# alshai/Big-BWT

Measured on AMD Instinct MI355X. Metric: input MB/s to .bwt (bit-exact vs ref), higher is better.
Workload: dtype u8; 1 GPU; BASELINE configs[2]: 64x mutated yeast-shaped FASTA (~0.79 GB), -w 10 -p 100, BWT + -s -e sampled SA; bytes_per_gpu=787308470, w=10, p=100, flags=6, phrases=16409159, words=921010, dict_bytes=79900101, parallelism=1 GPU

## Files before the change

big-bwt_amd/csrc/sufsort.hip:

```cpp
#include "kernels.hpp"
#include "prims.hpp"
#include "devutil.hpp"
#include <algorithm>
#include <cmath>
#include <optional>
#include <vector>
#include <cstdio>
#include <cstdlib>

namespace pfp {

enum : int { MODE_DICT = 0, MODE_PLAIN = 1 };

struct SufGeom {
  int mode; uint64_t N; WordView wv;
  const uint32_t *sym = nullptr;
  const uint32_t *dist = nullptr;
};
__device__ __forceinline__ uint64_t suf_len(const SufGeom &g, uint64_t i) {
  if (g.mode == MODE_DICT) return slen_of(g.wv, i) + 1;
  return g.N - i;
}

struct KeyCode {
// ... 529 lines not shown
#pragma unroll
      for (int s = 0; s < B; s++)
        if ((uint32_t)s < steps && !done) {
          const uint32_t qs = q + 4 * (uint32_t)s;
          differ(qs, X[s].x, Y[s].x); differ(qs + 1, X[s].y, Y[s].y); differ(qs + 2, X[s].z, Y[s].z); differ(qs + 3, X[s].w, Y[s].w);
        }
      q += 4 * steps;
    }
  }
  key[a] = k;
  val[a] = (I)i;
}
template <class I>
__global__ void heads64seg_kernel(uint64_t m, const uint8_t *__restrict__ gs, const uint64_t *__restrict__ key,
                                  const I *__restrict__ aslot, uint8_t *__restrict__ hd, I *__restrict__ hv) {
  uint64_t a = (uint64_t)BID * blockDim.x + threadIdx.x;
  if (a >= m) return;
  bool h = gs[a] || key[a] != key[a - 1];
  hd[a] = h ? 1 : 0;
  hv[a] = h ? aslot[a] : (I)0;
}
__global__ void rare_marks_kernel(const uint32_t *__restrict__ s, uint32_t N, const uint32_t *__restrict__ occ, uint32_t n_sym,
                                  uint32_t below, uint32_t *__restrict__ v) {
  uint32_t j = BID * blockDim.x + threadIdx.x;
  if (j >= N) return;
  const uint32_t x = s[N - 1 - j];
  const bool rare = x == 0 || x > n_sym || occ[x - 1] < below;
  v[j] = rare ? j + 1 : 0u;
}
__global__ void rare_dist_kernel(uint32_t N, const uint32_t *__restrict__ pm, uint32_t *__restrict__ dist) {
  uint32_t i = BID * blockDim.x + threadIdx.x;
  if (i >= N) return;
  const uint32_t j = N - 1 - i, mk = pm[j];
  dist[i] = mk ? j + 1 - mk : 0xFFFFFFFFu;
}

constexpr int kTile = 256;
__global__ __launch_bounds__(256) void active_count_kernel(const uint8_t *__restrict__ keep, const uint8_t *__restrict__ hd,
                                                           uint64_t m, uint32_t *__restrict__ tile_keep,
                                                           uint32_t *__restrict__ tile_heads) {
  const uint64_t t = (uint64_t)BID * 256 + threadIdx.x;
  const uint64_t base = t * 16;
  uint32_t k[4] = {0, 0, 0, 0}, h[4] = {0, 0, 0, 0};
  if (base < m) { load_flags16(keep, base, m, k); load_flags16(hd, base, m, h); }
  uint32_t ck = __popc(k[0]) + __popc(k[1]) + __popc(k[2]) + __popc(k[3]);
  uint32_t ch = __popc(k[0] & h[0]) + __popc(k[1] & h[1]) + __popc(k[2] & h[2]) + __popc(k[3] & h[3]);
#pragma unroll
  for (int o = 8; o > 0; o >>= 1) { ck += __shfl_down(ck, o, 16); ch += __shfl_down(ch, o, 16); }
  if ((threadIdx.x & 15) == 0 && base < m) { tile_keep[t >> 4] = ck; tile_heads[t >> 4] = ch; }
}
template <class I>
__global__ __launch_bounds__(256) void active_place_kernel(const uint8_t *__restrict__ keep, uint64_t m,
                                                           const uint32_t *__restrict__ tile_keep,
                                                           const I *__restrict__ tile_off,
                                                           const I *__restrict__ aslot, const I *__restrict__ val,
                                                           const I *__restrict__ newhead, I finbit,
                                                           I *__restrict__ aslot2, I *__restrict__ act_i,
                                                           I *__restrict__ act_grp) {
  __shared__ uint32_t ws[4];
  if ((uint64_t)BID * kTile >= m) return;
  if (tile_keep[BID] == 0) return;
  const uint64_t a = (uint64_t)BID * kTile + threadIdx.x;
  const bool k = a < m && keep[a];
  const unsigned long long mask = __ballot(k);
  const int lane = threadIdx.x & 63, wv = threadIdx.x >> 6;
  if (lane == 0) ws[wv] = (uint32_t)__popcll(mask);
  __syncthreads();
  if (!k) return;
  I pos = tile_off[BID] + (I)__popcll(mask & ((1ull << lane) - 1ull));
  for (int q = 0; q < wv; q++) pos += ws[q];
  aslot2[pos] = aslot ? aslot[a] : (I)a; act_i[pos] = val[a] & ~finbit; act_grp[pos] = newhead[a];
}

template <class I, class K>
__global__ void heads_kernel(uint64_t m, const K *__restrict__ key, const I *__restrict__ aslot,
                             uint8_t *__restrict__ hd, I *__restrict__ hv) {
  uint64_t a = (uint64_t)BID * blockDim.x + threadIdx.x;
  if (a >= m) return;
  bool h = (a == 0) || key[a] != key[a - 1];
  hd[a] = h ? 1 : 0;
  hv[a] = h ? aslot[a] : (I)0;
}

template <class I>
__global__ __launch_bounds__(256) void heads0_kernel(uint64_t m, const uint64_t *__restrict__ key, uint64_t keymask, int shift,
                                                     uint32_t T, uint8_t *__restrict__ hd, I *__restrict__ tile_last,
                                                     I *__restrict__ tab) {
  __shared__ I wl[4];
  if ((uint64_t)BID * 256 >= m) return;
  const uint64_t a = (uint64_t)BID * 256 + threadIdx.x;
  bool h = false;
  if (a < m) {
    const uint64_t k = key[a] & keymask, kprev = a ? (key[a - 1] & keymask) : ~k;
    h = k != kprev;
    hd[a] = h ? 1 : 0;
    if (a == 0 || (k >> shift) != (kprev >> shift)) tab[T - 1 - (uint32_t)(k >> shift)] = IdxTraits<I>::kNone - (I)a;
  }
  const unsigned long long mask = __ballot(h);
  if ((threadIdx.x & 63) == 0)
    wl[threadIdx.x >> 6] = mask ? (I)(BID * 256ull + (threadIdx.x & ~63) + (63 - __clzll((long long)mask))) : (I)0;
  __syncthreads();
  if (threadIdx.x == 0) {
    I v = wl[0];
    for (int q = 1; q < 4; q++) v = wl[q] > v ? wl[q] : v;
    tile_last[BID] = v;
  }
}
template <class I>
__global__ void fill_kernel(I *p, uint64_t n, I v) {
  uint64_t i = (uint64_t)BID * blockDim.x + threadIdx.x;
  if (i < n) p[i] = v;
}
template <class I>
__global__ __launch_bounds__(256) void write_back0_kernel(uint64_t m, const I *__restrict__ val,
                                                          const I *__restrict__ tile_scan,
                                                          const uint8_t *__restrict__ hd, const uint64_t *__restrict__ key0,
                                                          I *__restrict__ rank,
                                                          I *__restrict__ grp, uint8_t *__restrict__ keep, int write_ranks) {
  __shared__ I wl[4];
  if ((uint64_t)BID * 256 >= m) return;
  const uint64_t a = (uint64_t)BID * 256 + threadIdx.x;
  const int lane = threadIdx.x & 63, wv = threadIdx.x >> 6;
  const bool in = a < m;
  const bool h = in && hd[a];
  const bool hnext = in && (a + 1 == m || hd[a + 1]);
  const I i = in ? val[a] : (I)0;
  const uint32_t flagbit = in ? (uint32_t)(key0[a] & 1ull) : 0u;
  const I carry = BID ? tile_scan[BID - 1] : (I)0;
  const unsigned long long mask = __ballot(h);
  const I wbase = (I)(BID * 256ull + (threadIdx.x & ~63));
  if (lane == 0) wl[wv] = mask ? wbase + (63 - __clzll((long long)mask)) : (I)0;
  __syncthreads();
  if (!in) return;
  const unsigned long long upto = mask & (~0ull >> (63 - lane));
  I head;
  if (upto) head = wbase + (63 - __clzll((long long)upto));
  else {
    head = carry;
    for (int q = 0; q < wv; q++) head = wl[q] > head ? wl[q] : head;
  }
  grp[a] = head;
  const bool single = h && hnext;
  const bool fin = !single && flagbit;
  const bool k = !single && !fin;
  if (k && write_ranks) rank[i] = head;
  keep[a] = k ? 1 : 0;
}

template <class I>
__global__ void scatter_settled_kernel(uint64_t N, const I *__restrict__ sa, const I *__restrict__ grp,
                                       const uint8_t *__restrict__ keep, I finbit, I *__restrict__ rank) {
  uint64_t t = (uint64_t)BID * blockDim.x + threadIdx.x;
  if (t < N && !keep[t]) rank[sa[t]] = grp[t] | finbit;
}

constexpr int kPivBits = 23;
constexpr uint32_t kPivEq = 1u << 21;
constexpr uint32_t kPivCapMax = 8192;
template <class I>
__global__ void build_keys_pivot_kernel(const uint8_t *__restrict__ s, uint64_t m, uint64_t from, uint32_t cap,
                                        const I *__restrict__ act_i, const I *__restrict__ act_grp,
                                        const I *__restrict__ sa, I finbit, uint64_t *__restrict__ key,
                                        uint32_t *__restrict__ key32, I *__restrict__ val, int both = 0) {
  uint64_t a = (uint64_t)BID * blockDim.x + threadIdx.x;
  if (a >= m) return;
  const I i = act_i[a], grp = act_grp[a];
  const I piv = sa[grp];
  uint32_t ok = kPivEq;
  I settled = finbit;
  if (i != piv) {
    settled = 0;
    const uint8_t *pa = s + i + from, *pp = s + piv + from;
    uint32_t off = 0;
    uint4 xa0, xa1, xp0, xp1;
    bool hit = false;
    for (; off < cap; off += 32) {
      xa0 = ld16u(pa + off); xa1 = ld16u(pa + off + 16); xp0 = ld16u(pp + off); xp1 = ld16u(pp + off + 16);
      const uint32_t diff = (xa0.x ^ xp0.x) | (xa0.y ^ xp0.y) | (xa0.z ^ xp0.z) | (xa0.w ^ xp0.w) | (xa1.x ^ xp1.x) |
                            (xa1.y ^ xp1.y) | (xa1.z ^ xp1.z) | (xa1.w ^ xp1.w);
      const uint32_t term = lt2_flags32(xa0.x) | lt2_flags32(xa0.y) | lt2_flags32(xa0.z) | lt2_flags32(xa0.w) | lt2_flags32(xa1.x) |
                            lt2_flags32(xa1.y) | lt2_flags32(xa1.z) | lt2_flags32(xa1.w);
      if (diff | term) { hit = true; break; }
    }
    if (hit) {
      const uint64_t x[4] = {(uint64_t)xa0.x | ((uint64_t)xa0.y << 32), (uint64_t)xa0.z | ((uint64_t)xa0.w << 32),
                             (uint64_t)xa1.x | ((uint64_t)xa1.y << 32), (uint64_t)xa1.z | ((uint64_t)xa1.w << 32)};
      const uint64_t y[4] = {(uint64_t)xp0.x | ((uint64_t)xp0.y << 32), (uint64_t)xp0.z | ((uint64_t)xp0.w << 32),
                             (uint64_t)xp1.x | ((uint64_t)xp1.y << 32), (uint64_t)xp1.z | ((uint64_t)xp1.w << 32)};
      bool done = false;
#pragma unroll
      for (int q = 0; q < 4 && !done; q++) {
        const uint64_t tb = lt2_flags64(x[q]);
        if (x[q] == y[q]) { if (tb) { settled = finbit; done = true; } continue; }
        const int fd = __builtin_ctzll(x[q] ^ y[q]) >> 3;
        const int ft = tb ? (__builtin_ctzll(tb) >> 3) : 8;
        if (ft < fd) { settled = finbit; done = true; continue; }
        const uint32_t bx = (uint32_t)(x[q] >> (8 * fd)) & 0xffu, by = (uint32_t)(y[q] >> (8 * fd)) & 0xffu;
        const uint32_t lcp = off + 8 * q + fd;
        ok = bx < by ? ((lcp << 8) | bx) : ((2u << 21) | ((kPivCapMax - 1 - lcp) << 8) | bx);
        if (bx <= kEndOfWord) settled = finbit;
        done = true;
      }
    }
  }
  if (key32) key32[a] = ok;
  if (!key32 || both) key[a] = ((uint64_t)grp << kPivBits) | ok;
  val[a] = i | settled;
}
template <class I>
__global__ void veto_clear_kernel(uint64_t m, const I *__restrict__ newhead, uint8_t *__restrict__ veto) {
  uint64_t a = (uint64_t)BID * blockDim.x + threadIdx.x;
  if (a < m) veto[newhead[a]] = 0;
}
template <class I>
__global__ void pivot_veto_kernel(uint64_t m, const uint64_t *__restrict__ key, const uint32_t *__restrict__ key32,
                                  const I *__restrict__ val, const I *__restrict__ newhead, I finbit,
                                  uint8_t *__restrict__ veto) {
  uint64_t a = (uint64_t)BID * blockDim.x + threadIdx.x;
  if (a >= m) return;
  const uint32_t ok = key32 ? key32[a] : ((uint32_t)key[a] & ((1u << kPivBits) - 1));
  if (ok == kPivEq && !(val[a] & finbit)) veto[newhead[a]] = 1;
}

template <class I, class K>
__global__ void write_back_kernel(SufGeom g, uint64_t m, uint64_t sorted_len, const I *__restrict__ aslot,
                                  const I *__restrict__ val, const I *__restrict__ newhead,
                                  const uint8_t *__restrict__ hd, I finbit, const K *__restrict__ prevkey,
                                  int prevshift, const I *__restrict__ prevgrp, const uint8_t *__restrict__ veto,
                                  const uint32_t *__restrict__ wstart_bits, I *__restrict__ sa,
                                  I *__restrict__ rank, I *__restrict__ wordrank, I *__restrict__ grp, uint8_t *__restrict__ keep) {
  uint64_t a = (uint64_t)BID * blockDim.x + threadIdx.x;
  if (a >= m) return;
  const I iv = val[a], i = iv & ~finbit;
  const I slot = aslot[a];
  sa[slot] = i;
  grp[slot] = newhead[a];
// ... 38 lines not shown
                                    const I *__restrict__ sa, const I *__restrict__ grp, I finbit,
                                    I *__restrict__ rank) {
  uint64_t t = (uint64_t)BID * blockDim.x + threadIdx.x;
  if (t < N && refined[t] && !active[t]) rank[sa[t]] = grp[t] | finbit;
}

constexpr uint64_t kFinishMax = 1u << 17;
constexpr int kFinishGrp = 64;
constexpr uint32_t kFinishCmp = 8192;
__device__ __forceinline__ int finish_cmp_dict(const uint8_t *__restrict__ s, uint64_t i, uint64_t j, uint32_t *ovf) {
  for (uint32_t k = 0; k < kFinishCmp; k += 8) {
    const int r = cmp_term8(ld8u(s + i + k), ld8u(s + j + k));
    if (r != kCmpOn) return r;
  }
  *ovf = 1;
  return 0;
}
__device__ __forceinline__ int finish_cmp_int(const uint32_t *__restrict__ sym, uint64_t i, uint64_t j, uint32_t *ovf) {
  for (uint32_t k = 0; k < kFinishCmp / 4; k++) {
    const uint32_t x = sym[i + k], y = sym[j + k];
    if (x != y) return x < y ? -1 : 1;
  }
  *ovf = 1;
  return 0;
}
template <class I>
__global__ void finish_rank_kernel(SufGeom g, const uint8_t *__restrict__ s, uint64_t m, const I *__restrict__ act_i,
                                   const I *__restrict__ act_grp, uint32_t *__restrict__ lt, uint32_t *__restrict__ eq,
                                   uint32_t *__restrict__ gstart, uint32_t *__restrict__ overflow) {
  const uint64_t t = (uint64_t)BID * blockDim.x + threadIdx.x;
  const uint64_t a = t >> 3;
  const int l8 = (int)(t & 7);
  if (a >= m) return;
  const I grp = act_grp[a];
  uint64_t gs = a, ge = a + 1;
  while (gs > 0 && a - gs < (uint64_t)kFinishGrp && act_grp[gs - 1] == grp) gs--;
  while (ge < m && ge - gs <= (uint64_t)kFinishGrp && act_grp[ge] == grp) ge++;
  if (ge - gs > (uint64_t)kFinishGrp || (gs > 0 && act_grp[gs - 1] == grp)) { if (l8 == 0) atomicOr(overflow, 1u); return; }
  const uint64_t ia = act_i[a];
  uint32_t nlt = 0, neq = 0, ovf = 0;
  for (uint64_t b = gs + (uint64_t)l8; b < ge; b += 8) {
    if (b == a) continue;
    if (*(volatile uint32_t *)overflow) break;
    const uint64_t ib = act_i[b];
    const int cmp = g.mode == MODE_DICT ? finish_cmp_dict(s, ib, ia, &ovf) : finish_cmp_int(g.sym, ib, ia, &ovf);
    if (cmp < 0) nlt++;
    else if (cmp == 0 && b < a) neq++;
  }
  uint32_t packed = nlt | (neq << 8) | (ovf << 16);
  packed += __shfl_xor(packed, 1, 64); packed += __shfl_xor(packed, 2, 64); packed += __shfl_xor(packed, 4, 64);
  if (l8 != 0) return;
  if (packed >> 16) atomicOr(overflow, 1u);
  lt[a] = packed & 0xffu; eq[a] = (packed >> 8) & 0xffu; gstart[a] = (uint32_t)gs;
}
template <class I>
__global__ void finish_write_kernel(SufGeom g, uint64_t m, const I *__restrict__ aslot, const I *__restrict__ act_i, const uint32_t *__restrict__ lt,
                                    const uint32_t *__restrict__ eq, const uint32_t *__restrict__ gstart, I finbit,
                                    I *__restrict__ sa, I *__restrict__ grp, I *__restrict__ rank, I *__restrict__ wordrank) {
  const uint64_t a = (uint64_t)BID * blockDim.x + threadIdx.x;
  if (a >= m) return;
  const uint64_t gs = gstart[a];
  const I i = act_i[a], slot = aslot[gs + lt[a] + eq[a]], head = aslot[gs + lt[a]];
  sa[slot] = i;
  grp[slot] = head;
  if (rank) rank[i] = head | finbit;
  else if (wordrank && ((uint64_t)i == 0 || g.wv.bytes[(uint64_t)i - 1] == kEndOfWord)) wordrank[word_of(g.wv, i)] = head | finbit;
}

constexpr uint32_t kPivotAvg = 1024u;

constexpr uint64_t kLazyRatio = 8ull;

constexpr uint32_t kSegMinAvg = 24u;

struct SorterSwitches {
  bool lib_sort = getenv("PFP_OWN_SORT") == nullptr;
  bool finflag = getenv("PFP_NO_FINFLAG") == nullptr;
  bool finisher = getenv("PFP_NO_FINISHER") == nullptr;
  bool small_seg = getenv("PFP_NO_SMALLSEG") == nullptr;
  bool trace_rounds = getenv("PFP_TRACE_ROUNDS") != nullptr;
  uint32_t pivot_cap = []() { const char *e = getenv("PFP_PIVOT_CAP"); uint32_t v = e ? (uint32_t)atoll(e) : 512u; return v > kPivCapMax ? kPivCapMax : v; }();
};
static const SorterSwitches kSwitch;

template <class I>
RankViewT<I> rank_view(const SuffixOrderT<I> &so) {
  return RankViewT<I>{so.rank.p, so.skeys.p, so.tab.p, so.lut.p, so.bytes, so.N, so.kbits, so.shift, so.T, so.finbit, so.keymask, so.wordrank.p};
}
template RankViewT<uint32_t> rank_view(const SuffixOrderT<uint32_t> &);
template RankViewT<uint64_t> rank_view(const SuffixOrderT<uint64_t> &);

struct DoublingOpts {
  int key_bits = 64;
  bool dict = false;
  std::optional<uint64_t> list_len;
  bool whole_list = false;
  int idx_bits = 0;
};

enum class Round {
  FirstDict,
  FirstPlain,
  DictPivotGlobal,
  DictPivotGrouped,
  ParsePivot,
  DoublingGlobal,
  DoublingGrouped,
};

template <class I>
struct Rounds {
  using K = typename IdxTraits<I>::DKey;
  static constexpr bool kWide = sizeof(I) == 8;
  static constexpr int TB = 256;

  pfp_ctx *const c;
  const SufGeom g;
  SuffixOrderT<I> &out;
  const DoublingOpts o;
  const uint64_t NP, N;
  const bool lazy;
  const bool list_mode;
  const bool range_mode;
  const int nb;
  bool lazy_active = false, late_rank = false;
  I *rank_p = nullptr, *wordrank_p = nullptr;

  Round kind;
  uint64_t m, h, m2 = 0, ngrp = 0;
  uint32_t piv_cap = kSwitch.pivot_cap;
  bool pivot_ok = true;
  bool ipiv_ok = true;
  bool small_failed = false;
  bool finisher_ok = true;
  bool rank_alloc = false;
  bool lazy_pending = false;
  bool ranks_stale = false;
  bool active_stale = false;

  DBuf<uint64_t> &key;
  DBuf<I> &val;
  DBuf<I> tile_last, tile_scan;
  DBuf<uint64_t> keyo;
  DBuf<I> valo;
  DBuf<uint8_t> hd, keep;
  DBuf<I> aslot, aslot2, hv, newhead, act_i, act_grp;
  uint64_t list_cap = 0;
  DBuf<uint32_t> tile_keep, tile_heads;
  DBuf<I> tile_off, tile_hoff;
  DBuf<uint8_t> keep0, veto;
  DBuf<uint32_t> wstart_bits;
  DBuf<uint8_t> gs, bigf;
  DBuf<uint32_t> k32, k32o, segb, sege, nseg_d, ovf_d;
  DBuf<uint64_t> nsel_d;
  DBuf<K> dkey, dkeyo;

  Rounds(pfp_ctx *c_, const SufGeom &g_, DBuf<uint64_t> &key_, DBuf<I> &val_, uint64_t h0, SuffixOrderT<I> &out_, const DoublingOpts &o_)
      : c(c_), g(g_), out(out_), o(o_), NP(g_.N), N(o_.list_len.value_or(g_.N)), lazy(o_.dict), list_mode(o_.list_len.has_value()),
        range_mode(o_.list_len.has_value() && !o_.whole_list),
        nb(bits_for(N)), kind(o_.dict ? Round::FirstDict : Round::FirstPlain), m(N), h(h0), key(key_), val(val_) {}

  static uint64_t blocks(uint64_t n) { return cdiv(n, TB); }

  void first_round_sort() {
    keyo.alloc(c, N); valo.alloc(c, N);
    SortTag first_tag(g.mode == MODE_DICT ? "dictionary, first round" : "parse, first round");
    if (o.idx_bits) {
      if (kSwitch.lib_sort) sort_keys_db(c, key, keyo, N, o.idx_bits, o.idx_bits + o.key_bits);
      else msd_sort_keys_db(c, key, keyo, N, o.idx_bits, o.idx_bits + o.key_bits);
      KScope ks(c, "pfp::split_keys_kernel", N * (16 + sizeof(I)));
      hipLaunchKernelGGL(split_keys_kernel<I>, gdim(blocks(N)), gdim(TB), 0, c->stream, key.p, N, o.idx_bits, keyo.p, valo.p);
    } else {
      if (kSwitch.lib_sort) sort_pairs_db(c, key, keyo, val, valo, N, 0, o.key_bits);
      else msd_sort_pairs_db<I>(c, key, keyo, val, valo, N, 0, o.key_bits);
      std::swap(key, keyo); std::swap(val, valo);
    }
  }

  void alloc_lists(uint64_t cap) {
    aslot.alloc(c, cap); aslot2.alloc(c, cap); hv.alloc(c, cap); newhead.alloc(c, cap); act_i.alloc(c, cap); act_grp.alloc(c, cap);
    list_cap = cap;
  }
  void alloc_rank() {
    out.rank.alloc(c, NP);
    if (lazy) PFP_HIP(hipMemsetAsync(out.rank.p, 0xff, NP * sizeof(I), c->stream));
    rank_p = out.rank.p; rank_alloc = true;
  }

  void start_rounds() {
    if (lazy) { key.release(); val.release(); }
    hd.alloc(c, N + 1); keep.alloc(c, N);
    out.grp.alloc(c, N + 8);
    if (!lazy) {
      out.sa.alloc(c, N);
      alloc_lists(N);
      hipLaunchKernelGGL(iota_kernel<I>, gdim(blocks(N)), gdim(TB), 0, c->stream, aslot.p, N);
    } else {
      const int tb = std::min(o.key_bits, std::max(8, std::min(24, bits_for(N) - 5)));
      out.shift = o.key_bits - tb;
      out.T = 1u << tb;
      out.tab.alloc(c, out.T);
      hipLaunchKernelGGL(fill_kernel<I>, gdim(blocks(out.T)), gdim(TB), 0, c->stream, out.tab.p, (uint64_t)out.T,
                         (I)(IdxTraits<I>::kNone - (I)N));
    }
    out.finbit = (g.mode == MODE_DICT && (kWide || NP < (1ull << 31)) && kSwitch.finflag) ? IdxTraits<I>::kTop : (I)0;
    lazy_active = lazy && pivot_rounds_possible();
    late_rank = !range_mode && lazy_active && !c->debug;
    if (!range_mode && !late_rank) alloc_rank();
    if (late_rank) {
      out.wordrank.alloc(c, (uint64_t)g.wv.d + 1);
      PFP_HIP(hipMemsetAsync(out.wordrank.p, 0xff, ((uint64_t)g.wv.d + 1) * sizeof(I), c->stream));
      wordrank_p = out.wordrank.p;
    }
  }
  bool pivot_rounds_possible() const {
    return g.mode == MODE_DICT && out.finbit && kSwitch.pivot_cap >= 16 && (uint64_t)nb + kPivBits <= 64;
  }

  template <class KT>
  void heads(const KT *keys, int bytes) {
    KScope ks(c, "pfp::heads_kernel", m * bytes);
    hipLaunchKernelGGL((heads_kernel<I, KT>), gdim(blocks(m)), gdim(TB), 0, c->stream, m, keys, aslot.p, hd.p, hv.p);
  }
  void heads_k32() {
    KScope ks(c, "pfp::heads32_kernel", m * 14);
    hipLaunchKernelGGL(heads32_kernel<I>, gdim(blocks(m)), gdim(TB), 0, c->stream, m, gs.p, k32o.p, aslot.p, hd.p, hv.p);
  }

  void first_dict_heads_and_write_back() {
    tile_last.alloc(c, cdiv64(m, 256)); tile_scan.alloc(c, cdiv64(m, 256));
    { KScope ks(c, "pfp::heads0_kernel", m * 13);
      hipLaunchKernelGGL(heads0_kernel<I>, gdim(blocks(m)), gdim(TB), 0, c->stream, m, keyo.p, out.keymask, out.shift, out.T,
                         hd.p, tile_last.p, out.tab.p); }
    inclusive_max<I>(c, out.tab.p, out.tab.p, out.T);
    inclusive_max<I>(c, tile_last.p, tile_scan.p, cdiv64(m, 256));
    { KScope ks(c, "pfp::write_back0_kernel", m * (4 + 4 + 1 + 8 + 4 + 1));
      hipLaunchKernelGGL(write_back0_kernel<I>, gdim(blocks(m)), gdim(TB), 0, c->stream, m, valo.p, tile_scan.p, hd.p, keyo.p,
                         rank_p, out.grp.p, keep.p, (lazy_active || range_mode) ? 0 : 1); }
    if (lazy_active) active_stale = true;
    out.skeys = std::move(keyo);
    out.sa = std::move(valo);
  }

  void heads_and_write_back() {
    const uint64_t *keys = nullptr;
    const K *dkeys = nullptr;
    const I *prevgrp = nullptr;
    const uint32_t *pivk32 = nullptr;
    bool pivot = false;
    switch (kind) {
      case Round::FirstDict: return first_dict_heads_and_write_back();
      case Round::FirstPlain: heads(keyo.p, 17); break;
      case Round::DictPivotGlobal: heads(keyo.p, 17); keys = keyo.p; pivot = true; break;
      case Round::DictPivotGrouped: heads_k32(); prevgrp = act_grp.p; pivk32 = k32o.p; pivot = true; break;
      case Round::ParsePivot: {
        KScope ks(c, "pfp::heads64seg_kernel", m * 18);
        hipLaunchKernelGGL(heads64seg_kernel<I>, gdim(blocks(m)), gdim(TB), 0, c->stream, m, gs.p, keyo.p, aslot.p, hd.p, hv.p);
        prevgrp = act_grp.p;
      } break;
      case Round::DoublingGlobal:
        if constexpr (kWide) { heads(dkeyo.p, 25); dkeys = dkeyo.p; }
        else { heads(keyo.p, 17); keys = keyo.p; }
        break;
      case Round::DoublingGrouped: heads_k32(); prevgrp = act_grp.p; break;
    }
    inclusive_max<I>(c, hv.p, newhead.p, m);
    if (pivot) {
      if (!veto.p) veto.alloc(c, N);
      hipLaunchKernelGGL(veto_clear_kernel<I>, gdim(blocks(m)), gdim(TB), 0, c->stream, m, newhead.p, veto.p);
      hipLaunchKernelGGL(pivot_veto_kernel<I>, gdim(blocks(m)), gdim(TB), 0, c->stream, m, keyo.p, pivk32, valo.p, newhead.p, out.finbit, veto.p);
    }
    KScope ks(c, "pfp::write_back_kernel", m * (13 + 4 + 13));
    if (pivot && !wstart_bits.p) {
      wstart_bits.alloc(c, cdiv64(NP, 32));
      hipLaunchKernelGGL(word_start_bits_kernel, gdim(blocks(cdiv64(NP, 32))), gdim(TB), 0, c->stream, out.bytes, NP, wstart_bits.p);
    }
    const uint8_t *vetop = pivot ? veto.p : (const uint8_t *)nullptr;
    const uint32_t *lazyb = pivot ? wstart_bits.p : (const uint32_t *)nullptr;
    if (dkeys)
      hipLaunchKernelGGL((write_back_kernel<I, K>), gdim(blocks(m)), gdim(TB), 0, c->stream, g, m, h, aslot.p, valo.p, newhead.p, hd.p,
                         out.finbit, dkeys, nb, prevgrp, vetop, lazyb, out.sa.p, rank_p, wordrank_p, out.grp.p, keep.p);
    else
      hipLaunchKernelGGL((write_back_kernel<I, uint64_t>), gdim(blocks(m)), gdim(TB), 0, c->stream, g, m, h, aslot.p, valo.p, newhead.p,
                         hd.p, out.finbit, keys, pivot ? kPivBits : nb, prevgrp, vetop, lazyb, out.sa.p, rank_p, wordrank_p, out.grp.p, keep.p);
    if (pivot) { ranks_stale = true; active_stale = true; }
  }

  void compact() {
    const bool round0 = kind == Round::FirstDict;
    const uint64_t ntile = cdiv64(m, kTile);
    if (!tile_keep.p) { tile_keep.alloc(c, cdiv64(N, kTile) + 1); tile_heads.alloc(c, cdiv64(N, kTile) + 1);
                        tile_off.alloc(c, cdiv64(N, kTile) + 1); tile_hoff.alloc(c, cdiv64(N, kTile) + 1); }
    auto read_counts = [&]() {
      sync(c);
      I t0, t1;
      memcpy(&t0, c->h_scalars, sizeof(I)); memcpy(&t1, c->h_scalars + 1, sizeof(I));
      m2 = t0; ngrp = t1;
    };
    {
      PFP_HIP(hipMemsetAsync(tile_keep.p + ntile, 0, 4, c->stream));
      PFP_HIP(hipMemsetAsync(tile_heads.p + ntile, 0, 4, c->stream));
      KScope ks(c, "pfp::active_place_kernel", m * 2 + 0);
      hipLaunchKernelGGL(active_count_kernel, gdim((unsigned)cdiv64(ntile, 16)), gdim(256), 0, c->stream, keep.p, hd.p, m,
                         tile_keep.p, tile_heads.p);
      exclusive_sum_u32_to<I>(c, tile_keep.p, tile_off.p, ntile + 1);
      exclusive_sum_u32_to<I>(c, tile_heads.p, tile_hoff.p, ntile + 1);
      PFP_HIP(hipMemcpyAsync(c->h_scalars, tile_off.p + ntile, sizeof(I), hipMemcpyDeviceToHost, c->stream));
      PFP_HIP(hipMemcpyAsync(c->h_scalars + 1, tile_hoff.p + ntile, sizeof(I), hipMemcpyDeviceToHost, c->stream));
      if (round0) {
        read_counts();
        if (m2) alloc_lists(m2);
      }
      if (!round0 || m2)
        hipLaunchKernelGGL(active_place_kernel<I>, gdim((unsigned)ntile), gdim(256), 0, c->stream, keep.p, m, tile_keep.p, tile_off.p,
                           round0 ? (const I *)nullptr : aslot.p, round0 ? out.sa.p : valo.p, round0 ? out.grp.p : newhead.p, out.finbit,
                           aslot2.p, act_i.p, act_grp.p);
      PFP_HIP(hipGetLastError());
    }
    if (!round0) read_counts();
  }

  void regroup() {
    heads_and_write_back();
    compact();
    if (kind == Round::FirstDict && m2) {
      lazy_pending = true;
      keep0.alloc(c, N);
      PFP_HIP(hipMemcpyAsync(keep0.p, keep.p, N, hipMemcpyDeviceToDevice, c->stream));
      out.n_refined = m2;
      if (out.paybits) {
        out.refined.alloc(c, N + 16);
        PFP_HIP(hipMemcpyAsync(out.refined.p, keep.p, N, hipMemcpyDeviceToDevice, c->stream));
        PFP_HIP(hipMemsetAsync(out.refined.p + N, 0, 16, c->stream));
      }
    }
    if (kSwitch.trace_rounds) {
      const bool grouped = kind == Round::DictPivotGrouped || kind == Round::ParsePivot || kind == Round::DoublingGrouped;
      fprintf(stderr, "[pfp] doubling N=%llu round=%llu h=%llu m=%llu -> %llu unresolved in %llu groups%s\n", (unsigned long long)N,
              (unsigned long long)out.rounds, (unsigned long long)h, (unsigned long long)m, (unsigned long long)m2,
              (unsigned long long)ngrp, grouped ? " (seg)" : (kind == Round::DictPivotGlobal ? " (pivot)" : ""));
    }
  }

  void judge_pivot_round() {
    if (kind == Round::ParsePivot && m2 * 4 > m) ipiv_ok = false;
    if ((kind == Round::DictPivotGlobal || kind == Round::DictPivotGrouped) && m2 * 2 > m) {
      const uint32_t next_cap = std::min<uint32_t>(piv_cap * 4, kPivCapMax - 16);
      if (piv_cap < kPivCapMax - 16 && piv_cap >= 16 && m2 * (uint64_t)next_cap < N * 128) piv_cap = next_cap;
      else pivot_ok = false;
    }
  }

  void next_list() {
    std::swap(aslot, aslot2);
    m = m2;
    if (m == 0) return;
    PFP_REQUIRE(h < 2 * NP, PFP_EHIP, "suffix sort failed to converge");
    if (!keyo.p || keyo.n < m) keyo.alloc(c, m);
    if (!key.p || key.n < m) key.alloc(c, m);
    if (!valo.p || valo.n < m) valo.alloc(c, m);
    if (!val.p || val.n < m) val.alloc(c, m);
  }

  bool try_finisher() {
    if (!(kSwitch.finisher && finisher_ok && m <= kFinishMax && out.rounds >= 1 && (g.mode == MODE_DICT || (g.mode == MODE_PLAIN && g.sym))))
      return false;
    DBuf<uint32_t> flt(c, m), feq(c, m), fgs(c, m), fov(c, 1);
    fov.zero();
    KScope ks(c, "pfp::finish_rank_kernel", m * (sizeof(I) * 4 + 12));
    hipLaunchKernelGGL(finish_rank_kernel<I>, gdim(blocks(m * 8)), gdim(TB), 0, c->stream, g, out.bytes, m, act_i.p, act_grp.p, flt.p, feq.p,
                       fgs.p, fov.p);
    if (read_scalar(c, fov.p) != 0) {
      finisher_ok = false;
      return false;
    }
    { KScope kw(c, "pfp::finish_write_kernel", m * (sizeof(I) * 5 + 12));
      hipLaunchKernelGGL(finish_write_kernel<I>, gdim(blocks(m)), gdim(TB), 0, c->stream, g, m, aslot.p, act_i.p, flt.p, feq.p, fgs.p,
                         out.finbit, out.sa.p, out.grp.p, rank_p, wordrank_p); }
    PFP_HIP(hipGetLastError());
    if (kSwitch.trace_rounds) fprintf(stderr, "[pfp] doubling N=%llu round=%llu: the last %llu suffixes ranked by comparison\n",
                                      (unsigned long long)N, (unsigned long long)out.rounds, (unsigned long long)m);
    out.rounds++;
    m = 0;
    return true;
  }


  bool small_groups() const {
    return kSwitch.small_seg && ngrp && m / ngrp <= (kWide ? kSmallSeg / 4 : kSmallSeg / 2) && (!small_failed || m / ngrp <= 3);
  }
  bool segmented_worthwhile() const { return ngrp && m >= (1u << 20) && m < 0xFFFFFFFFull && m / ngrp >= kSegMinAvg; }

  void seg_bufs() {
    if (!gs.p) { gs.alloc(c, list_cap + 1); k32.alloc(c, list_cap); k32o.alloc(c, list_cap); nseg_d.alloc(c, 2); nsel_d.alloc(c, 1); ovf_d.alloc(c, 1); }
  }
  template <class KT>
  bool place_small_groups(const KT *kin, KT *kout) {
    constexpr bool side = !kWide && sizeof(KT) == 4;
    seg_bufs();
    ovf_d.zero();
    if (side && (!bigf.p || bigf.n < m + 16)) bigf.alloc(c, list_cap + 16);
    { KScope ks(c, "pfp::seg_small_sort_kernel", m * (2 * sizeof(KT) + 3 * sizeof(I) + 1));
      hipLaunchKernelGGL((seg_small_sort_kernel<I, KT>), gdim(blocks(m)), gdim(TB), 0, c->stream, m, act_grp.p, kin, val.p, gs.p, kout,
                         valo.p, ovf_d.p, side ? bigf.p : (uint8_t *)nullptr); }
    if (read_scalar(c, ovf_d.p) == 0) return true;
    if (!side) return false;
    PFP_HIP(hipMemsetAsync(bigf.p + m, 0, 16, c->stream));
    const uint64_t nbig = count_flags(c, bigf.p, m);
    if (nbig * 2 > m) return false;
    DBuf<I> idx(c, nbig + 1), sv(c, nbig), sva(c, nbig);
    DBuf<uint64_t> sk(c, nbig), ska(c, nbig), cnt(c, 1);
    select_index<I>(c, bigf.p, idx.p, cnt.p, m);
    hipLaunchKernelGGL(big_seg_gather_kernel<I>, gdim(blocks(nbig)), gdim(TB), 0, c->stream, nbig, idx.p, act_grp.p, k32o.p, valo.p, sk.p, sv.p);
    sort_pairs_db(c, sk, ska, sv, sva, nbig, 0, 32 + nb);
    hipLaunchKernelGGL(big_seg_scatter_kernel<I>, gdim(blocks(nbig)), gdim(TB), 0, c->stream, nbig, idx.p, sk.p, sv.p, k32o.p, valo.p);
    PFP_HIP(hipGetLastError());
    return true;
  }
  bool library_segments() {
    seg_bufs();
    if (!segb.p) { segb.alloc(c, list_cap + 1); sege.alloc(c, list_cap + 1); }
    hipLaunchKernelGGL(group_starts_kernel<I>, gdim(blocks(m)), gdim(TB), 0, c->stream, m, act_grp.p, gs.p);
    select_index<uint32_t>(c, gs.p, segb.p, nsel_d.p, m);
    PFP_HIP(hipMemsetAsync(nseg_d.p + 1, 0, 4, c->stream));
    if (c->debug) PFP_REQUIRE(read_scalar(c, nsel_d.p) == ngrp, PFP_EHIP, "group count of the active list differs from the compaction's");
    hipLaunchKernelGGL(seg_end_kernel, gdim(blocks(ngrp)), gdim(TB), 0, c->stream, (uint32_t)ngrp, (uint32_t)m, segb.p, sege.p, nseg_d.p + 1);
    return read_scalar(c, nseg_d.p + 1) <= (1u << 15);
  }
  void sort_device_wide(int bits) {
    sort_pairs_db(c, key, keyo, val, valo, m, 0, bits);
    std::swap(key, keyo); std::swap(val, valo);
  }

  bool dict_pivot_wanted() const { return pivot_ok && pivot_rounds_possible() && ngrp && m / ngrp <= kPivotAvg; }
  void dict_pivot_round() {
    if (piv_cap >= 16 && piv_cap < kPivCapMax - 16 && out.rounds >= 2 && m * (uint64_t)(kPivCapMax - 16) < N * 128) piv_cap = kPivCapMax - 16;
    bool small = small_groups();
    bool seg = !small && segmented_worthwhile() && library_segments();
    if (small) seg_bufs();
    { KScope ks(c, "pfp::build_keys_pivot_kernel", m * (4 + 4 + 4 + 12 + 64));
      hipLaunchKernelGGL(build_keys_pivot_kernel<I>, gdim(blocks(m)), gdim(TB), 0, c->stream, out.bytes, m, h, piv_cap, act_i.p,
                         act_grp.p, out.sa.p, out.finbit, key.p, (seg || small) ? k32.p : (uint32_t *)nullptr, val.p, small ? 1 : 0); }
    if (small && !place_small_groups(k32.p, k32o.p)) {
      small = false; small_failed = true;
      seg = segmented_worthwhile() && library_segments();
    }
    if (seg) segsort_pairs_u32<I>(c, k32.p, k32o.p, val.p, valo.p, m, (uint32_t)ngrp, segb.p, sege.p, 0, kPivBits);
    else if (!small) sort_device_wide(nb + kPivBits);
    kind = (small || seg) ? Round::DictPivotGrouped : Round::DictPivotGlobal;
    out.rounds++;
  }

  bool parse_pivot_wanted() const {
    return g.mode == MODE_PLAIN && g.dist && g.sym && ipiv_ok && ngrp && (range_mode || m >= parse_pivot_min()) && m < 0xFFFFFFFFull && m / ngrp >= 2;
  }
  bool parse_pivot_round() {
    {
      DBuf<unsigned long long> best(c, N);
      best.zero();
      KScope ks(c, "pfp::ipivot_keys_kernel", m * (4 + 4 + 4 + 8 + 16 + 12 + 64));
      const bool batched = ipivot_batched();
      uint32_t *dvs = batched ? reinterpret_cast<uint32_t *>(hv.p) : nullptr;
      hipLaunchKernelGGL(ipivot_select_kernel<I>, gdim(blocks(m)), gdim(TB), 0, c->stream, m, NP, h, act_i.p, act_grp.p, g.dist, best.p, dvs);
      if (batched)
        hipLaunchKernelGGL((ipivot_keys_batch_kernel<I, kIntPivBatch>), gdim(blocks(m)), gdim(TB), 0, c->stream, m, NP, h, kIntPivCap, g.sym,
                           act_i.p, act_grp.p, best.p, dvs, key.p, val.p);
      else
        hipLaunchKernelGGL(ipivot_keys_kernel<I>, gdim(blocks(m)), gdim(TB), 0, c->stream, m, NP, h, kIntPivCap, g.sym, act_i.p,
                           act_grp.p, best.p, key.p, val.p);
    }
    bool sorted = m / ngrp <= kSmallSeg / 2 && place_small_groups(key.p, keyo.p);
    if (!sorted && (m / ngrp >= 4 || range_mode) && library_segments()) {
      segsort_pairs_u64_u32(c, key.p, keyo.p, val.p, valo.p, m, (uint32_t)ngrp, segb.p, sege.p, 0, 32 + bits_for(2 * kIntPivCap + 3));
      sorted = true;
    }
    if (!sorted) { ipiv_ok = false; return false; }
    kind = Round::ParsePivot;
    out.rounds++;
    return true;
  }

  void repair_ranks(uint64_t m_active, const I *aslot_list) {
    if (!ranks_stale) return;
    DBuf<uint8_t> act(c, N);
    act.zero();
    if (m_active) hipLaunchKernelGGL(mark_slots_kernel<I>, gdim(blocks(m_active)), gdim(TB), 0, c->stream, m_active, aslot_list, act.p);
    KScope ks(c, "pfp::repair_ranks_kernel", N * 6);
    hipLaunchKernelGGL(repair_ranks_kernel<I>, gdim(blocks(N)), gdim(TB), 0, c->stream, N, keep0.p, act.p, out.sa.p, out.grp.p,
                       out.finbit, out.rank.p);
    ranks_stale = false;
  }
  void prepare_ranks_for_doubling() {
    if (late_rank && !rank_alloc) {
      alloc_rank();
      ranks_stale = true;
    }
    if (lazy_pending) {
      lazy_pending = false;
      if (m * kLazyRatio > N) {
        KScope ks(c, "pfp::scatter_settled_kernel", N * (4 + 4 + 1 + 4));
        hipLaunchKernelGGL(scatter_settled_kernel<I>, gdim(blocks(N)), gdim(TB), 0, c->stream, N, out.sa.p, out.grp.p, keep0.p,
                           out.finbit, out.rank.p);
        if (!out.paybits) out.skeys.release();
        out.tab.release();
      }
    }
    repair_ranks(m, aslot.p);
    if (active_stale) {
      hipLaunchKernelGGL(active_ranks_kernel<I>, gdim(blocks(m)), gdim(TB), 0, c->stream, m, act_i.p, act_grp.p, out.rank.p);
      active_stale = false;
    }
  }

  void build_keys32(const RankViewT<I> &L) {
    KScope ks(c, "pfp::build_keys32_kernel", m * (4 + 4 + 8));
    hipLaunchKernelGGL(build_keys32_kernel, gdim(blocks(m)), gdim(TB), 0, c->stream, g, m, h, act_i.p, L, k32.p, val.p);
  }
  void doubling_round() {
    const RankViewT<I> L = rank_view(out);
    const int keybits = 2 * nb;
    kind = Round::DoublingGlobal;
    if constexpr (kWide) {
      if (!dkey.p || dkey.n < m) { dkey.alloc(c, m); dkeyo.alloc(c, m); }
      { KScope ks(c, "pfp::build_keys_kernel", m * (8 + 8 + 8 + 24));
        hipLaunchKernelGGL(build_keys_kernel<I>, gdim(blocks(m)), gdim(TB), 0, c->stream, g, m, h, act_i.p, act_grp.p, L, nb, dkey.p, val.p); }
      sort_pairs_db(c, dkey, dkeyo, val, valo, m, 0, keybits);
      std::swap(dkey, dkeyo); std::swap(val, valo);
    } else {
      if (small_groups()) {
        seg_bufs();
        build_keys32(L);
        if (place_small_groups(k32.p, k32o.p)) kind = Round::DoublingGrouped;
        else small_failed = true;
      }
      if (kind != Round::DoublingGrouped && segmented_worthwhile() && library_segments()) {
        build_keys32(L);
        segsort_pairs_u32<I>(c, k32.p, k32o.p, val.p, valo.p, m, (uint32_t)ngrp, segb.p, sege.p, 0, bits_for(N));
        kind = Round::DoublingGrouped;
      }
      if (kind != Round::DoublingGrouped) {
        { KScope ks(c, "pfp::build_keys_kernel", m * (4 + 4 + 4 + 12));
          hipLaunchKernelGGL(build_keys_kernel<I>, gdim(blocks(m)), gdim(TB), 0, c->stream, g, m, h, act_i.p, act_grp.p, L, nb, key.p, val.p); }
        sort_device_wide(keybits);
      }
    }
    h *= 2;
    out.rounds++;
  }

  bool next_round() {
    if (dict_pivot_wanted()) { dict_pivot_round(); return true; }
    if constexpr (!kWide) {
      if (parse_pivot_wanted() && parse_pivot_round()) return true;
    }
    if (list_mode) { out.complete = false; return false; }
    prepare_ranks_for_doubling();
    doubling_round();
    return true;
  }
};

template <class I>
static void doubling(pfp_ctx *c, SufGeom g, DBuf<uint64_t> &key, DBuf<I> &val, uint64_t h0, SuffixOrderT<I> &out, const DoublingOpts &o) {
  Rounds<I> r(c, g, key, val, h0, out, o);
  out.N = r.N; out.NP = r.NP; out.range = r.range_mode; out.complete = true;
  out.rounds = 0;
  if (r.N == 0) { out.sa.alloc(c, 1); out.grp.alloc(c, 8); out.rank.alloc(c, 1); return; }
  r.first_round_sort();
  SortTag later_tag(g.mode == MODE_DICT ? "dictionary, later rounds" : "parse, later rounds");
  r.start_rounds();
  for (;;) {
    r.regroup();
    r.judge_pivot_round();
    r.next_list();
    if (r.m == 0 || r.try_finisher() || !r.next_round()) break;
// ... 523 lines not shown
```

Measured before the change: 31400 MB/s.

## Fold tile keep/head counts into first-round write-back and defer plain rank allocation

The first-round write_back kernel now also computes per-tile keep and head counts via ballots, so the separate active_count pass is skipped in round 0 for both dict and plain modes. Plain mode gets a specialized heads/write-back path that avoids the iota and full active-list setup. It also delays rank allocation until doubling, filling it from the slots then. In dict mode the keep buffer is moved into keep0 instead of copied. These cut extra passes over N-sized arrays and device memory traffic, at the cost of more template specializations and env-switch paths that could diverge in correctness.

```diff
diff --git a/big-bwt_amd/csrc/sufsort.hip b/big-bwt_amd/csrc/sufsort.hip
--- a/big-bwt_amd/csrc/sufsort.hip
+++ b/big-bwt_amd/csrc/sufsort.hip
@@ -635,7 +635,7 @@
   hv[a] = h ? aslot[a] : (I)0;
 }
 
-template <class I>
+template <class I, bool DICT>
 __global__ __launch_bounds__(256) void heads0_kernel(uint64_t m, const uint64_t *__restrict__ key, uint64_t keymask, int shift,
                                                      uint32_t T, uint8_t *__restrict__ hd, I *__restrict__ tile_last,
                                                      I *__restrict__ tab) {
@@ -644,10 +644,14 @@
   const uint64_t a = (uint64_t)BID * 256 + threadIdx.x;
   bool h = false;
   if (a < m) {
-    const uint64_t k = key[a] & keymask, kprev = a ? (key[a - 1] & keymask) : ~k;
-    h = k != kprev;
+    if constexpr (DICT) {
+      const uint64_t k = key[a] & keymask, kprev = a ? (key[a - 1] & keymask) : ~k;
+      h = k != kprev;
+      if (a == 0 || (k >> shift) != (kprev >> shift)) tab[T - 1 - (uint32_t)(k >> shift)] = IdxTraits<I>::kNone - (I)a;
+    } else {
+      h = a == 0 || key[a] != key[a - 1];
+    }
     hd[a] = h ? 1 : 0;
-    if (a == 0 || (k >> shift) != (kprev >> shift)) tab[T - 1 - (uint32_t)(k >> shift)] = IdxTraits<I>::kNone - (I)a;
   }
   const unsigned long long mask = __ballot(h);
   if ((threadIdx.x & 63) == 0)
@@ -664,13 +668,15 @@
   uint64_t i = (uint64_t)BID * blockDim.x + threadIdx.x;
   if (i < n) p[i] = v;
 }
-template <class I>
+template <class I, bool DICT>
 __global__ __launch_bounds__(256) void write_back0_kernel(uint64_t m, const I *__restrict__ val,
                                                           const I *__restrict__ tile_scan,
                                                           const uint8_t *__restrict__ hd, const uint64_t *__restrict__ key0,
                                                           I *__restrict__ rank,
-                                                          I *__restrict__ grp, uint8_t *__restrict__ keep, int write_ranks) {
+                                                          I *__restrict__ grp, uint8_t *__restrict__ keep, int write_ranks,
+                                                          uint32_t *__restrict__ tile_keep, uint32_t *__restrict__ tile_heads) {
   __shared__ I wl[4];
+  __shared__ uint32_t wk[4], wh[4];
   if ((uint64_t)BID * 256 >= m) return;
   const uint64_t a = (uint64_t)BID * 256 + threadIdx.x;
   const int lane = threadIdx.x & 63, wv = threadIdx.x >> 6;
@@ -678,12 +684,24 @@
   const bool h = in && hd[a];
   const bool hnext = in && (a + 1 == m || hd[a + 1]);
   const I i = in ? val[a] : (I)0;
-  const uint32_t flagbit = in ? (uint32_t)(key0[a] & 1ull) : 0u;
+  uint32_t flagbit = 0u;
+  if constexpr (DICT) flagbit = in ? (uint32_t)(key0[a] & 1ull) : 0u;
   const I carry = BID ? tile_scan[BID - 1] : (I)0;
   const unsigned long long mask = __ballot(h);
   const I wbase = (I)(BID * 256ull + (threadIdx.x & ~63));
+  const bool single = h && hnext;
+  const bool fin = !single && flagbit;
+  const bool k = in && !single && !fin;
   if (lane == 0) wl[wv] = mask ? wbase + (63 - __clzll((long long)mask)) : (I)0;
+  if (tile_keep) {
+    const unsigned long long km = __ballot(k), khm = __ballot(k && h);
+    if (lane == 0) { wk[wv] = (uint32_t)__popcll(km); wh[wv] = (uint32_t)__popcll(khm); }
+  }
   __syncthreads();
+  if (tile_keep && threadIdx.x == 0) {
+    tile_keep[BID] = wk[0] + wk[1] + wk[2] + wk[3];
+    tile_heads[BID] = wh[0] + wh[1] + wh[2] + wh[3];
+  }
   if (!in) return;
   const unsigned long long upto = mask & (~0ull >> (63 - lane));
   I head;
@@ -693,10 +711,11 @@
     for (int q = 0; q < wv; q++) head = wl[q] > head ? wl[q] : head;
   }
   grp[a] = head;
-  const bool single = h && hnext;
-  const bool fin = !single && flagbit;
-  const bool k = !single && !fin;
-  if (k && write_ranks) rank[i] = head;
+  if constexpr (DICT) {
+    if (k && write_ranks) rank[i] = head;
+  } else {
+    if (rank) rank[i] = head;
+  }
   keep[a] = k ? 1 : 0;
 }
 
@@ -704,7 +723,7 @@
 __global__ void scatter_settled_kernel(uint64_t N, const I *__restrict__ sa, const I *__restrict__ grp,
                                        const uint8_t *__restrict__ keep, I finbit, I *__restrict__ rank) {
   uint64_t t = (uint64_t)BID * blockDim.x + threadIdx.x;
-  if (t < N && !keep[t]) rank[sa[t]] = grp[t] | finbit;
+  if (t < N && !(keep && keep[t])) rank[sa[t]] = grp[t] | finbit;
 }
 
 constexpr int kPivBits = 23;
@@ -909,6 +928,7 @@
   uint32_t pivot_cap = []() { const char *e = getenv("PFP_PIVOT_CAP"); uint32_t v = e ? (uint32_t)atoll(e) : 512u; return v > kPivCapMax ? kPivCapMax : v; }();
 };
 static const SorterSwitches kSwitch;
+static bool switch_on(const char *name) { const char *e = getenv(name); return !e || atoi(e) != 0; }
 
 template <class I>
 RankViewT<I> rank_view(const SuffixOrderT<I> &so) {
@@ -950,7 +970,9 @@
   const bool list_mode;
   const bool range_mode;
   const int nb;
+  const bool plain_lazy, plain_tiles, dict_fold;
   bool lazy_active = false, late_rank = false;
+  bool plain_late = false;
   I *rank_p = nullptr, *wordrank_p = nullptr;
 
   Round kind;
@@ -985,7 +1007,10 @@
   Rounds(pfp_ctx *c_, const SufGeom &g_, DBuf<uint64_t> &key_, DBuf<I> &val_, uint64_t h0, SuffixOrderT<I> &out_, const DoublingOpts &o_)
       : c(c_), g(g_), out(out_), o(o_), NP(g_.N), N(o_.list_len.value_or(g_.N)), lazy(o_.dict), list_mode(o_.list_len.has_value()),
         range_mode(o_.list_len.has_value() && !o_.whole_list),
-        nb(bits_for(N)), kind(o_.dict ? Round::FirstDict : Round::FirstPlain), m(N), h(h0), key(key_), val(val_) {}
+        nb(bits_for(N)), plain_lazy(!o_.dict && switch_on("PFP_PLAIN_LAZY_RANK")), plain_tiles(!o_.dict && switch_on("PFP_PLAIN_TILES")),
+        dict_fold(o_.dict && switch_on("PFP_DICT_FOLD")), kind(o_.dict ? Round::FirstDict : Round::FirstPlain), m(N), h(h0), key(key_),
+        val(val_) {}
+  bool tiles_first() const { return lazy || plain_tiles; }
 
   static uint64_t blocks(uint64_t n) { return cdiv(n, TB); }
 
@@ -1019,9 +1044,11 @@
     hd.alloc(c, N + 1); keep.alloc(c, N);
     out.grp.alloc(c, N + 8);
     if (!lazy) {
-      out.sa.alloc(c, N);
-      alloc_lists(N);
-      hipLaunchKernelGGL(iota_kernel<I>, gdim(blocks(N)), gdim(TB), 0, c->stream, aslot.p, N);
+      if (!plain_tiles) {
+        out.sa.alloc(c, N);
+        alloc_lists(N);
+        hipLaunchKernelGGL(iota_kernel<I>, gdim(blocks(N)), gdim(TB), 0, c->stream, aslot.p, N);
+      }
     } else {
       const int tb = std::min(o.key_bits, std::max(8, std::min(24, bits_for(N) - 5)));
       out.shift = o.key_bits - tb;
@@ -1033,7 +1060,8 @@
     out.finbit = (g.mode == MODE_DICT && (kWide || NP < (1ull << 31)) && kSwitch.finflag) ? IdxTraits<I>::kTop : (I)0;
     lazy_active = lazy && pivot_rounds_possible();
     late_rank = !range_mode && lazy_active && !c->debug;
-    if (!range_mode && !late_rank) alloc_rank();
+    plain_late = !lazy && !range_mode && plain_lazy && !c->debug;
+    if (!range_mode && !late_rank && !plain_late) alloc_rank();
     if (late_rank) {
       out.wordrank.alloc(c, (uint64_t)g.wv.d + 1);
       PFP_HIP(hipMemsetAsync(out.wordrank.p, 0xff, ((uint64_t)g.wv.d + 1) * sizeof(I), c->stream));
@@ -1054,18 +1082,38 @@
     hipLaunchKernelGGL(heads32_kernel<I>, gdim(blocks(m)), gdim(TB), 0, c->stream, m, gs.p, k32o.p, aslot.p, hd.p, hv.p);
   }
 
+  bool counts_from_write_back() const { return lazy ? dict_fold : plain_tiles; }
+  void alloc_tile_counts() {
+    if (!tile_keep.p) { tile_keep.alloc(c, cdiv64(N, kTile) + 1); tile_heads.alloc(c, cdiv64(N, kTile) + 1);
+                        tile_off.alloc(c, cdiv64(N, kTile) + 1); tile_hoff.alloc(c, cdiv64(N, kTile) + 1); }
+  }
   void first_dict_heads_and_write_back() {
+    const bool counts = counts_from_write_back();
+    if (counts) alloc_tile_counts();
     tile_last.alloc(c, cdiv64(m, 256)); tile_scan.alloc(c, cdiv64(m, 256));
     { KScope ks(c, "pfp::heads0_kernel", m * 13);
-      hipLaunchKernelGGL(heads0_kernel<I>, gdim(blocks(m)), gdim(TB), 0, c->stream, m, keyo.p, out.keymask, out.shift, out.T,
+      hipLaunchKernelGGL((heads0_kernel<I, true>), gdim(blocks(m)), gdim(TB), 0, c->stream, m, keyo.p, out.keymask, out.shift, out.T,
                          hd.p, tile_last.p, out.tab.p); }
     inclusive_max<I>(c, out.tab.p, out.tab.p, out.T);
     inclusive_max<I>(c, tile_last.p, tile_scan.p, cdiv64(m, 256));
     { KScope ks(c, "pfp::write_back0_kernel", m * (4 + 4 + 1 + 8 + 4 + 1));
-      hipLaunchKernelGGL(write_back0_kernel<I>, gdim(blocks(m)), gdim(TB), 0, c->stream, m, valo.p, tile_scan.p, hd.p, keyo.p,
-                         rank_p, out.grp.p, keep.p, (lazy_active || range_mode) ? 0 : 1); }
+      hipLaunchKernelGGL((write_back0_kernel<I, true>), gdim(blocks(m)), gdim(TB), 0, c->stream, m, valo.p, tile_scan.p, hd.p, keyo.p,
+                         rank_p, out.grp.p, keep.p, (lazy_active || range_mode) ? 0 : 1,
+                         counts ? tile_keep.p : (uint32_t *)nullptr, counts ? tile_heads.p : (uint32_t *)nullptr); }
     if (lazy_active) active_stale = true;
     out.skeys = std::move(keyo);
+    out.sa = std::move(valo);
+  }
+  void first_plain_heads_and_write_back() {
+    alloc_tile_counts();
+    tile_last.alloc(c, cdiv64(m, 256)); tile_scan.alloc(c, cdiv64(m, 256));
+    { KScope ks(c, "pfp::heads0_kernel", m * 9);
+      hipLaunchKernelGGL((heads0_kernel<I, false>), gdim(blocks(m)), gdim(TB), 0, c->stream, m, keyo.p, ~0ull, 0, 0u, hd.p, tile_last.p,
+                         (I *)nullptr); }
+    inclusive_max<I>(c, tile_last.p, tile_scan.p, cdiv64(m, 256));
+    { KScope ks(c, "pfp::write_back0_kernel", m * (sizeof(I) + 1 + sizeof(I) + 1 + (rank_p ? sizeof(I) : 0)));
+      hipLaunchKernelGGL((write_back0_kernel<I, false>), gdim(blocks(m)), gdim(TB), 0, c->stream, m, valo.p, tile_scan.p, hd.p,
+                         (const uint64_t *)nullptr, rank_p, out.grp.p, keep.p, 0, tile_keep.p, tile_heads.p); }
     out.sa = std::move(valo);
   }
 
@@ -1077,7 +1125,10 @@
     bool pivot = false;
     switch (kind) {
       case Round::FirstDict: return first_dict_heads_and_write_back();
-      case Round::FirstPlain: heads(keyo.p, 17); break;
+      case Round::FirstPlain:
+        if (plain_tiles) return first_plain_heads_and_write_back();
+        heads(keyo.p, 17);
+        break;
       case Round::DictPivotGlobal: heads(keyo.p, 17); keys = keyo.p; pivot = true; break;
       case Round::DictPivotGrouped: heads_k32(); prevgrp = act_grp.p; pivk32 = k32o.p; pivot = true; break;
       case Round::ParsePivot: {
@@ -1114,10 +1165,9 @@
   }
 
   void compact() {
-    const bool round0 = kind == Round::FirstDict;
+    const bool round0 = kind == Round::FirstDict || (kind == Round::FirstPlain && plain_tiles);
     const uint64_t ntile = cdiv64(m, kTile);
-    if (!tile_keep.p) { tile_keep.alloc(c, cdiv64(N, kTile) + 1); tile_heads.alloc(c, cdiv64(N, kTile) + 1);
-                        tile_off.alloc(c, cdiv64(N, kTile) + 1); tile_hoff.alloc(c, cdiv64(N, kTile) + 1); }
+    alloc_tile_counts();
     auto read_counts = [&]() {
       sync(c);
       I t0, t1;
@@ -1128,8 +1178,9 @@
       PFP_HIP(hipMemsetAsync(tile_keep.p + ntile, 0, 4, c->stream));
       PFP_HIP(hipMemsetAsync(tile_heads.p + ntile, 0, 4, c->stream));
       KScope ks(c, "pfp::active_place_kernel", m * 2 + 0);
-      hipLaunchKernelGGL(active_count_kernel, gdim((unsigned)cdiv64(ntile, 16)), gdim(256), 0, c->stream, keep.p, hd.p, m,
-                         tile_keep.p, tile_heads.p);
+      if (!(round0 && counts_from_write_back()))
+        hipLaunchKernelGGL(active_count_kernel, gdim((unsigned)cdiv64(ntile, 16)), gdim(256), 0, c->stream, keep.p, hd.p, m,
+                           tile_keep.p, tile_heads.p);
       exclusive_sum_u32_to<I>(c, tile_keep.p, tile_off.p, ntile + 1);
       exclusive_sum_u32_to<I>(c, tile_heads.p, tile_hoff.p, ntile + 1);
       PFP_HIP(hipMemcpyAsync(c->h_scalars, tile_off.p + ntile, sizeof(I), hipMemcpyDeviceToHost, c->stream));
@@ -1152,12 +1203,17 @@
     compact();
     if (kind == Round::FirstDict && m2) {
       lazy_pending = true;
-      keep0.alloc(c, N);
-      PFP_HIP(hipMemcpyAsync(keep0.p, keep.p, N, hipMemcpyDeviceToDevice, c->stream));
+      if (dict_fold) {
+        keep0 = std::move(keep);
+        keep.alloc(c, m2);
+      } else {
+        keep0.alloc(c, N);
+        PFP_HIP(hipMemcpyAsync(keep0.p, keep.p, N, hipMemcpyDeviceToDevice, c->stream));
+      }
       out.n_refined = m2;
       if (out.paybits) {
         out.refined.alloc(c, N + 16);
-        PFP_HIP(hipMemcpyAsync(out.refined.p, keep.p, N, hipMemcpyDeviceToDevice, c->stream));
+        PFP_HIP(hipMemcpyAsync(out.refined.p, keep0.p, N, hipMemcpyDeviceToDevice, c->stream));
         PFP_HIP(hipMemsetAsync(out.refined.p + N, 0, 16, c->stream));
       }
     }
@@ -1318,6 +1374,15 @@
     ranks_stale = false;
   }
   void prepare_ranks_for_doubling() {
+    if (plain_late && !rank_alloc) {
+      alloc_rank();
+      KScope ks(c, "pfp::scatter_settled_kernel", N * 3 * sizeof(I));
+      hipLaunchKernelGGL(scatter_settled_kernel<I>, gdim(blocks(N)), gdim(TB), 0, c->stream, N, out.sa.p, out.grp.p, (const uint8_t *)nullptr,
+                         (I)0, out.rank.p);
+      if (getenv("PFP_TRACE_ROUNDS"))
+        fprintf(stderr, "[pfp] doubling N=%llu round=%llu: rank[] allocated late and filled from the slots\n", (unsigned long long)N,
+                (unsigned long long)out.rounds + 1);
+    }
     if (late_rank && !rank_alloc) {
       alloc_rank();
       ranks_stale = true;
```

Result: faster. 32220 MB/s, median of 6 (+2.6%).
